# BIH-CEI/napkon-string-matching

Hardware: AMD Instinct MI355X
Metric: pair-comparisons/sec (whole node), N x M all-pairs (higher is better)
Workload: dtype u64; 1 GPU; C3: 200000x200000 strings/GPU (len U[16,64], 37 symbols), fuzzy_match RAW, threshold 0.8; score_func=fuzzy_match, mode=RAW, hits_per_rank=2000, hits_all_ranks=2000, exact_prune=True, hit_ordering=second stream, overlapped with the next step's grid kernel (two hit buffers)

## Files before the change

### napkon-string-matching_amd/csrc/indel_raw_coarse.hpp

```cpp
#pragma once

namespace nsm {

#ifndef NSM_C3C_CAP
#define NSM_C3C_CAP 3
#endif
#ifndef NSM_C3C_FP4
#define NSM_C3C_FP4 1
#endif
#ifndef NSM_C3C_FP4_PERM
#define NSM_C3C_FP4_PERM 1
#endif
#ifndef NSM_C3C_FP4_SPLIT
#define NSM_C3C_FP4_SPLIT 4
#endif
#ifndef NSM_C3C_NT
#define NSM_C3C_NT 4
#endif
#ifndef NSM_C3C_ORFOLD
#define NSM_C3C_ORFOLD (NSM_C3C_FP4 && NSM_C3C_NT % 2 == 0)
#endif
#ifndef NSM_C3C_PIPE
#define NSM_C3C_PIPE (NSM_C3C_NT % (NSM_C3C_ORFOLD ? 4 : 2) == 0)
#endif
#ifndef NSM_C3C_OR_SPLIT
#define NSM_C3C_OR_SPLIT 2
#endif
#ifndef NSM_C3C_LCS_PREFETCH
#define NSM_C3C_LCS_PREFETCH 1
#endif
#ifndef NSM_C3C_EARLY_OUT
#define NSM_C3C_EARLY_OUT 1
#endif
#ifndef NSM_C3C_PERSIST
#define NSM_C3C_PERSIST 0
#endif
#ifndef NSM_C3P_ITEM_ROWS
#define NSM_C3P_ITEM_ROWS 0
#endif
constexpr int kC3cBlock = 32;
constexpr int kC3cRights = NSM_C3C_NT * kC3cBlock;
constexpr int kC3cPipeExtra = NSM_C3C_PIPE ? (NSM_C3C_ORFOLD ? 2 : 1) : 0;
constexpr int kC3cStack = (NSM_C3C_NT + 2 + kC3cPipeExtra) * kWave;
constexpr int kC3cDrainAt = 2 * kWave;
static_assert(NSM_C3C_NT >= 1 && NSM_C3C_NT <= 4, "an entry keeps its tile in 2 bits");
static_assert(NSM_C3C_CAP >= 2 && NSM_C3C_CAP <= 8, "code slots per bucket");

static inline size_t c3c_lds_bytes() {
  return static_cast<size_t>(kWavesPerBlock) * (kC3cStack * 8 + static_cast<size_t>(kC3cRights) * (8 * 4 + 1)) + 136;
}

typedef int c3c_v4i __attribute__((ext_vector_type(4)));
typedef int c3c_v16i __attribute__((ext_vector_type(16)));
typedef int c3c_v8i __attribute__((ext_vector_type(8)));
typedef float c3c_v16f __attribute__((ext_vector_type(16)));

__device__ __forceinline__ uint32_t c3c_ge64(uint32_t w, int k) {
  return (w + static_cast<uint32_t>(0x40 - k) * 0x01010101u) & 0x40404040u;
}


__device__ __forceinline__ int c3c_fp4_scale(const uint4& f0, const uint4& f1) {
  const uint32_t ws[8] = {f0.x, f0.y, f0.z, f0.w, f1.x, f1.y, f1.z, f1.w};
  uint32_t any = 0u;
#pragma unroll
  for (int q = 0; q < 8; ++q) any |= ws[q];
  if ((any & 0xf0f0f0f0u) == 0u) return 0;
  uint32_t top = 0u;
#pragma unroll
  for (int q = 0; q < 8; ++q)
#pragma unroll
    for (int b = 0; b < 4; ++b) top = max(top, (ws[q] >> (8 * b)) & 0xffu);
  return top <= 27u ? 1 : top <= 51u ? 2 : 3;
}
__device__ __forceinline__ void c3c_fp4_right_k0(uint32_t fw, int& m1, int& m2) {
  const uint32_t sel = fw & 0x07070707u;
  const uint32_t big = ((fw >> 3) & 0x01010101u) * 0xffu;
  const uint32_t lo1 = __builtin_amdgcn_perm(0x11111111u, 0x11110100u, sel);
  const uint32_t lo2 = __builtin_amdgcn_perm(0x41312111u, 0x01000000u, sel), hi2 = __builtin_amdgcn_perm(0x71717171u, 0x61615151u, sel);
  m1 = static_cast<int>((big & 0x11111111u) | (~big & lo1));
  m2 = static_cast<int>((big & hi2) | (~big & lo2));
}
__device__ __forceinline__ void c3c_fp4_right_scaled(uint32_t fw, int k, int& m1, int& m2) {
  m1 = static_cast<int>((c3c_ge64(fw, 1) >> 6) | (c3c_ge64(fw, 2) >> 2));
  uint32_t w2 = c3c_ge64(fw, 3) >> 6;
  const uint32_t round_up = (1u << k) - 1u;
#pragma unroll
  for (int b = 0; b < 4; ++b) {
    const uint32_t r = (fw >> (8 * b)) & 0xffu;
    const uint32_t q = (max(r, 3u) - 3u + round_up) >> k;
    w2 |= (static_cast<uint32_t>(0x7777665543210ull >> (4u * q)) & 0xfu) << (8 * b + 4);
  }
  m2 = static_cast<int>(w2);
}
__device__ __forceinline__ void c3c_fp4_left(uint32_t w, int& m1, int& m2) {
#if NSM_C3C_FP4_PERM
  const uint32_t sel = (w + 0x3c3c3c3cu) & 0x43434343u;
  m1 = static_cast<int>(__builtin_amdgcn_perm(0u, 0x44440400u, sel) & 0x44444444u);
  m2 = static_cast<int>(__builtin_amdgcn_perm(0u, 0x04000000u, sel) & 0x44444444u);
#else
  m1 = static_cast<int>(((c3c_ge64(w, 1) >> 4)) | c3c_ge64(w, 2));
  m2 = static_cast<int>(((c3c_ge64(w, 3) >> 4)) | c3c_ge64(w, 4));
#endif
}
__device__ __forceinline__ c3c_v16f c3c_fp4_mfma1(const c3c_v4i& a, const c3c_v4i& b) {
  const c3c_v8i a8 = {a.x, a.y, a.z, a.w, 0, 0, 0, 0}, b8 = {b.x, b.y, b.z, b.w, 0, 0, 0, 0};
  const c3c_v16f zero = {0, 0, 0, 0, 0, 0, 0, 0, 0, 0, 0, 0, 0, 0, 0, 0};
  return __builtin_amdgcn_mfma_scale_f32_32x32x64_f8f6f4(a8, b8, zero, 4, 4, 0, 0, 0, 0);
}
__device__ __forceinline__ c3c_v16f c3c_fp4_mfma2(const c3c_v4i& a, const c3c_v4i& b, const c3c_v16f& acc, int scales, int t) {
  const c3c_v8i a8 = {a.x, a.y, a.z, a.w, 0, 0, 0, 0}, b8 = {b.x, b.y, b.z, b.w, 0, 0, 0, 0};
  switch (t) {
    case 0: return __builtin_amdgcn_mfma_scale_f32_32x32x64_f8f6f4(a8, b8, acc, 4, 4, 0, 0x7f7f7f7f, 0, scales);
    case 1: return __builtin_amdgcn_mfma_scale_f32_32x32x64_f8f6f4(a8, b8, acc, 4, 4, 0, 0x7f7f7f7f, 1, scales);
    case 2: return __builtin_amdgcn_mfma_scale_f32_32x32x64_f8f6f4(a8, b8, acc, 4, 4, 0, 0x7f7f7f7f, 2, scales);
    default: return __builtin_amdgcn_mfma_scale_f32_32x32x64_f8f6f4(a8, b8, acc, 4, 4, 0, 0x7f7f7f7f, 3, scales);
  }
}

constexpr int kC3cPackedRow = 64;
#ifndef NSM_C3C_PACK_MIN_PAIRS
#define NSM_C3C_PACK_MIN_PAIRS 10000000000ll
#endif
static inline bool c3c_pack_pays(long long pairs) { return pairs >= static_cast<long long>(NSM_C3C_PACK_MIN_PAIRS); }
struct c3c_packed_rows {
  c3c_v4i m1, m2;
};
template <bool PACKED>
struct c3c_rows {
  typedef uint4 type;
};
template <>
struct c3c_rows<true> {
  typedef c3c_packed_rows type;
};

__device__ __forceinline__ void c3c_pack_left_unit(const uint32_t* __restrict__ lhist, c3c_v4i* __restrict__ packed, int n_left,
                                                   int u) {
  if (u >= 2 * n_left) return;
  const uint4 w = reinterpret_cast<const uint4*>(lhist)[u];
  const uint32_t ws[4] = {w.x, w.y, w.z, w.w};
  c3c_v4i m1, m2;
#pragma unroll
  for (int q = 0; q < 4; ++q) {
    int a1, a2;
    c3c_fp4_left(ws[q], a1, a2);
    m1[q] = a1;
    m2[q] = a2;
  }
  packed[2 * static_cast<size_t>(u)] = m1;
  packed[2 * static_cast<size_t>(u) + 1] = m2;
}
__global__ __launch_bounds__(kBlock) void c3c_pack_left_kernel(const uint32_t* __restrict__ lhist, c3c_v4i* __restrict__ packed,
                                                               int n_left) {
  c3c_pack_left_unit(lhist, packed, n_left, blockIdx.x * kBlock + threadIdx.x);
}

constexpr int kC3pWindow = 1 << 15;
struct C3pItemParams {
  int n_left, n_right, n_tiles, item_rows, every_row;
  unsigned int cap;
  uint8_t la_lo[65], la_hi[65];
};
__host__ __device__ static inline int c3p_items_of(int rows, int item_rows) {
  const int per_window = (kC3pWindow + item_rows - 1) / item_rows;
  return (rows >> 15) * per_window + ((rows & (kC3pWindow - 1)) + item_rows - 1) / item_rows;
}
constexpr int kC3pQueueBytes = 64;
__host__ __device__ static inline unsigned int* c3p_queue(const char* lpacked) {
  return reinterpret_cast<unsigned int*>(const_cast<char*>(lpacked) - kC3pQueueBytes);
}
__host__ __device__ static inline int4* c3p_item(unsigned int* queue, unsigned int k) {
  return reinterpret_cast<int4*>(queue) - 1 - k;
}
__global__ __launch_bounds__(kBlock) void c3p_prepass_kernel(const uint32_t* __restrict__ lhist, c3c_v4i* __restrict__ packed,
                                                             const int32_t* __restrict__ rlen, const int32_t* __restrict__ lstart,
                                                             unsigned int* __restrict__ queue,
                                                             const C3pItemParams ip, int item_blocks) {
  if (static_cast<int>(blockIdx.x) >= item_blocks) {
    c3c_pack_left_unit(lhist, packed, ip.n_left, (static_cast<int>(blockIdx.x) - item_blocks) * kBlock + static_cast<int>(threadIdx.x));
    return;
  }
  __shared__ unsigned long long s_scan[kBlock];
  const int tid = threadIdx.x;
  auto interval = [&](int t, int& r0) -> int {
    r0 = 0;
    if (ip.every_row) return ip.n_left;
    const int j_a = t * kC3cRights, j_b = min(j_a + kC3cRights, ip.n_right) - 1;
    const int lb_a = min(max(rlen[j_a], 0), 64), lb_b = min(max(rlen[j_b], 0), 64);
    int lo = 65, hi = 0;
    for (int lb = min(lb_a, lb_b); lb <= max(lb_a, lb_b); ++lb) {
      lo = min(lo, static_cast<int>(ip.la_lo[lb]));
      hi = max(hi, static_cast<int>(ip.la_hi[lb]));
    }
    if (hi < lo) return 0;
    r0 = lstart[64 - hi];
    return lstart[64 - lo + 1] - r0;
  };
  unsigned int before = 0u;
  for (int t = tid; t < static_cast<int>(blockIdx.x) * kBlock; t += kBlock) {
    int r0;
    before += static_cast<unsigned int>(c3p_items_of(interval(t, r0), ip.item_rows));
  }
  const int tile = static_cast<int>(blockIdx.x) * kBlock + tid;
  int r0 = 0, rows = 0;
  if (tile < ip.n_tiles) rows = interval(tile, r0);
  const unsigned int own = static_cast<unsigned int>(c3p_items_of(rows, ip.item_rows));
  unsigned long long v = (static_cast<unsigned long long>(before) << 32) | own;
  s_scan[tid] = v;
  __syncthreads();
  for (int d = 1; d < kBlock; d <<= 1) {
    const unsigned long long add = tid >= d ? s_scan[tid - d] : 0ull;
    __syncthreads();
    v += add;
    s_scan[tid] = v;
    __syncthreads();
  }
  const unsigned long long total = s_scan[kBlock - 1];
  const unsigned int carry = static_cast<unsigned int>(total >> 32);
  unsigned int at = carry + static_cast<unsigned int>(v) - own;
  const int per_window = (kC3pWindow + ip.item_rows - 1) / ip.item_rows;
  for (unsigned int k = 0; k < own; ++k, ++at) {
    const int base = r0 + (static_cast<int>(k) / per_window) * kC3pWindow;
    const int first = base + (static_cast<int>(k) % per_window) * ip.item_rows;
    const int end = min(first + ip.item_rows, min(base + kC3pWindow, r0 + rows));
    if (at < ip.cap) *c3p_item(queue, at) = make_int4(tile, first, end, base);
  }
  if (static_cast<int>(blockIdx.x) == item_blocks - 1 && tid == 0) {
    queue[0] = 0u;
    queue[1] = min(carry + static_cast<unsigned int>(total), ip.cap);
  }
}

#ifndef NSM_C3C_OCC
#define NSM_C3C_OCC __attribute__((amdgpu_waves_per_eu((NSM_C3C_ORFOLD && PACKED) ? 4 : 2)))
#endif
template <int NT, int CAP, bool PACKED, bool PERSIST = false>
__global__ __launch_bounds__(kBlock) NSM_C3C_OCC void indel_raw_coarse_kernel(
    const uint8_t* __restrict__ lcodes, const int32_t* __restrict__ llen, const int32_t* __restrict__ lstart,
    const int32_t* __restrict__ lorig, const uint32_t* __restrict__ lhist, const uint8_t* __restrict__ rcodes,
    const int32_t* __restrict__ rlen, const int32_t* __restrict__ rorig, const uint32_t* __restrict__ rhist,
    nsm_hit* __restrict__ hits, unsigned long long* __restrict__ count, const IndelRawParams p,
    const char* __restrict__ lpacked) {
  static_assert(!PACKED || NSM_C3C_FP4, "only the FP4 scan has packed left rows");
  static_assert(!PERSIST || PACKED, "the persistent launch is the packed scan's");
  constexpr int kRights = NT * kC3cBlock;
  static_assert(kC3cDrainAt >= kWave && kC3cDrainAt + (NT + kC3cPipeExtra) * kWave <= kC3cStack,
                "the drain is triggered above kC3cDrainAt entries and runs full passes");
  constexpr bool kOrFold = NSM_C3C_ORFOLD && PACKED;
  constexpr int kFlagHi = 1 << 17, kFlagLo = 1 << 8;
  static_assert(!kOrFold || (NSM_C3C_FP4 && NT % 2 == 0), "the OR fold puts tiles 2 p and 2 p + 1 of the FP4 scan on one accumulator");
  extern __shared__ __attribute__((aligned(16))) unsigned long long s_mem[];
  unsigned long long* s_stack = s_mem;
  uint32_t* s_rh = reinterpret_cast<uint32_t*>(s_stack + kWavesPerBlock * kC3cStack);
  uint8_t* s_rl = reinterpret_cast<uint8_t*>(s_rh + kWavesPerBlock * 8 * kRights);
  uint8_t* s_lcsmin = s_rl + kWavesPerBlock * kRights;
  for (int t = threadIdx.x; t < 132; t += kBlock) s_lcsmin[t] = p.lcsmin[t];
  __syncthreads();

  const int lane = threadIdx.x & (kWave - 1);
  const int wave = threadIdx.x >> 6;
  const int col = lane & (kC3cBlock - 1);
  const int half = lane >> 5;
  int j0 = (blockIdx.x * kWavesPerBlock + wave) * kRights;
  if (!PERSIST && j0 >= p.n_right) return;
  auto lane_again = [&]() -> int {
    int l = lane;
    asm volatile("" : "+v"(l));
    return l;
  };
#if NSM_C3C_EARLY_OUT
  if (!PERSIST && p.zero_need != 0) {
    const int ie = blockIdx.y * p.rows_per_chunk;
    const int la_hi = llen[ie], la_lo = llen[min(p.n_left, ie + p.rows_per_chunk) - 1];
    bool fits = false;
#pragma unroll
    for (int k = 0; k < (kRights + kWave - 1) / kWave; ++k) {
      const int j = j0 + k * kWave + lane;
      if (k * kWave + lane < kRights && j < p.n_right) {
        const int lb = rlen[j];
        const int la = min(max(lb, la_lo), la_hi);
        const int nd = (la == 0 || lb == 0) ? p.zero_need : static_cast<int>(s_lcsmin[la + lb]);
        fits = fits || min(la, lb) >= nd;
      }
    }
    if (!__any(fits)) return;
  }
#endif
  unsigned long long* stack = s_stack + wave * kC3cStack;
  uint32_t* rh_lds = s_rh + wave * 8 * kRights;
  uint8_t* rl_lds = s_rl + wave * kRights;

  bool valid[NT];
  c3c_v4i bfrag[NT][NSM_C3C_FP4 ? 2 : CAP];
  uint32_t bscales = 0u;
  int q_cnt = 0;
  int i0 = 0, ifirst = 0, i1 = 0;
  int it_cur = 0, it_end = 0;
  bool other_tile = true;
  if constexpr (PERSIST) j0 = -1;
  do {
    if constexpr (PERSIST) {
      unsigned int* queue = c3p_queue(lpacked);
      if (it_cur >= it_end) {
        const unsigned int n_items = static_cast<unsigned int>(__builtin_amdgcn_readfirstlane(static_cast<int>(queue[1])));
        unsigned int start = 0u, grain = 0u;
        if (lane == 0) {
          const unsigned int seen = *reinterpret_cast<volatile unsigned int*>(queue);
          const unsigned int left = seen < n_items ? n_items - seen : 0u;
          grain = max(1u, left / (2u * gridDim.x * kWavesPerBlock));
          start = atomicAdd(queue, grain);
        }
        const unsigned int s = static_cast<unsigned int>(__builtin_amdgcn_readfirstlane(static_cast<int>(start)));
        const unsigned int g = static_cast<unsigned int>(__builtin_amdgcn_readfirstlane(static_cast<int>(grain)));
        if (s >= n_items) return;
        it_cur = static_cast<int>(s);
        it_end = static_cast<int>(min(s + g, n_items));
      }
      const int4 it = *c3p_item(queue, static_cast<unsigned int>(it_cur++));
      const int j_it = __builtin_amdgcn_readfirstlane(it.x) * kRights;
      other_tile = j_it != j0;
      j0 = j_it;
      ifirst = __builtin_amdgcn_readfirstlane(it.y);
      i1 = __builtin_amdgcn_readfirstlane(it.z);
      i0 = __builtin_amdgcn_readfirstlane(it.w);
    }
    if (!PERSIST || other_tile) {
      int ln = lane;
      if constexpr (PERSIST) ln = lane_again();
#pragma unroll
      for (int k = 0; k < (kRights + kWave - 1) / kWave; ++k) {
        const int rl = k * kWave + ln;
        if (rl < kRights) {
          const int j = j0 + rl;
          const int jcl = j < p.n_right ? j : p.n_right - 1;
          const uint4* fp = reinterpret_cast<const uint4*>(rhist + static_cast<size_t>(jcl) * 8);
          const uint4 f0 = fp[0], f1 = fp[1];
          uint32_t* dst = rh_lds + rl;
          dst[0 * kRights] = f0.x; dst[1 * kRights] = f0.y; dst[2 * kRights] = f0.z; dst[3 * kRights] = f0.w;
          dst[4 * kRights] = f1.x; dst[5 * kRights] = f1.y; dst[6 * kRights] = f1.z; dst[7 * kRights] = f1.w;
          rl_lds[rl] = static_cast<uint8_t>(j < p.n_right ? rlen[jcl] : 0);
        }
      }
    }
#if NSM_C3C_FP4
    auto scale_base = [](int t) -> uint32_t { return (kOrFold && t % 2 == 0) ? 0x7fu + 9u : 0x7fu; };
    uint32_t bscales1 = 0u;
    if constexpr (kOrFold) {
#pragma unroll
      for (int t = 0; t < NT; ++t) bscales1 |= scale_base(t) << (8 * t);
      asm volatile("" : "+v"(bscales1));
    }
    auto code_tile = [&](int t, const uint4& f, int k) __attribute__((always_inline)) {
      const uint32_t ws[4] = {f.x, f.y, f.z, f.w};
      if (k == 0) {
#pragma unroll
        for (int q = 0; q < 4; ++q) {
          int m1, m2;
          c3c_fp4_right_k0(ws[q], m1, m2);
          bfrag[t][0][q] = m1;
          bfrag[t][1][q] = m2;
        }
      } else {
#pragma unroll
        for (int q = 0; q < 4; ++q) {
          int m1, m2;
          c3c_fp4_right_scaled(ws[q], k, m1, m2);
          bfrag[t][0][q] = m1;
          bfrag[t][1][q] = m2;
        }
      }
    };
    if (!PERSIST || other_tile) {
      bscales = 0u;
      int col_r = col, half_r = half;
      if constexpr (PERSIST) {
        const int l = lane_again();
        col_r = l & (kC3cBlock - 1);
        half_r = l >> 5;
      }
#pragma unroll
      for (int t = 0; t < NT; ++t) {
        const int j = j0 + t * kC3cBlock + col_r;
        valid[t] = j < p.n_right;
        const int jcl = valid[t] ? j : p.n_right - 1;
        const uint4* fp = reinterpret_cast<const uint4*>(rhist + static_cast<size_t>(jcl) * 8);
        const uint4 f0 = fp[0], f1 = fp[1];
        const int k = c3c_fp4_scale(f0, f1);
        bscales |= (scale_base(t) + static_cast<uint32_t>(k)) << (8 * t);
        uint4 f = half_r ? f1 : f0;
        if (!valid[t]) f = make_uint4(0u, 0u, 0u, 0u);
        code_tile(t, f, k);
      }
    }
    auto make_bfrag = [&]() __attribute__((always_inline)) {
      const int l = lane_again();
      const uint32_t* rp0 = rh_lds + (4 * (l >> 5)) * kRights + (l & (kC3cBlock - 1));
#pragma unroll
      for (int t = 0; t < NT; ++t) {
        const uint32_t* rp = rp0 + t * kC3cBlock;
        const int k = static_cast<int>(((bscales >> (8 * t)) & 0xffu) - scale_base(t));
        uint4 f = make_uint4(rp[0], rp[kRights], rp[2 * kRights], rp[3 * kRights]);
        if (!valid[t]) f = make_uint4(0u, 0u, 0u, 0u);
        code_tile(t, f, k);
      }
    };
    __builtin_amdgcn_fence(__ATOMIC_ACQ_REL, "wavefront");
    __builtin_amdgcn_wave_barrier();
#else
    auto code_b = [&](int t, int q, uint32_t fw) {
      const uint32_t full = c3c_ge64(fw, CAP);
#pragma unroll
      for (int s = 0; s < CAP - 1; ++s)
        bfrag[t][s][q] = static_cast<int>((c3c_ge64(fw, s + 1) ^ full) >> 6);
      bfrag[t][CAP - 1][q] = static_cast<int>(full);
    };
#pragma unroll
    for (int t = 0; t < NT; ++t) {
      const int j = j0 + t * kC3cBlock + col;
      valid[t] = j < p.n_right;
      const int jcl = valid[t] ? j : p.n_right - 1;
      uint4 f = reinterpret_cast<const uint4*>(rhist + static_cast<size_t>(jcl) * 8)[half];
      if (!valid[t]) f = make_uint4(0u, 0u, 0u, 0u);
      code_b(t, 0, f.x); code_b(t, 1, f.y); code_b(t, 2, f.z); code_b(t, 3, f.w);
    }
    auto make_bfrag = [&]() {
#pragma unroll
      for (int t = 0; t < NT; ++t) {
        const uint32_t* rp = rh_lds + (4 * half) * kRights + t * kC3cBlock + col;
#pragma unroll
        for (int q = 0; q < 4; ++q) code_b(t, q, valid[t] ? rp[q * kRights] : 0u);
      }
    };
    __builtin_amdgcn_fence(__ATOMIC_ACQ_REL, "wavefront");
    __builtin_amdgcn_wave_barrier();
#endif
    if constexpr (!PERSIST) {
      i0 = ifirst = blockIdx.y * p.rows_per_chunk;
      i1 = min(p.n_left, i0 + p.rows_per_chunk);
    }

    auto need_of = [&](int la, int lb) -> int { return (la == 0 || lb == 0) ? p.zero_need : static_cast<int>(s_lcsmin[la + lb]); };

    const char* chunk = reinterpret_cast<const char*>(lhist + static_cast<size_t>(i0) * 8);
    const char* pchunk = PACKED ? lpacked + static_cast<size_t>(i0) * kC3cPackedRow : nullptr;

    auto drain_pass = [&]() __attribute__((always_inline)) {
      __builtin_amdgcn_fence(__ATOMIC_ACQ_REL, "wavefront");
      __builtin_amdgcn_wave_barrier();
      const int n = min(q_cnt, kWave);
      const int base = q_cnt - n;
      q_cnt = base;
#ifdef NSM_C3C_X_NODRAIN
      return;
#endif
      const int m = lane & 3;
      uint32_t mask = 0;
#pragma nounroll
      for (int s = (n - 1) >> 4; s >= 0; --s) {
        const int e = 16 * s + (lane >> 2);
        const bool active = e < n;
        const unsigned long long ent = stack[base + (active ? e : 0)];
        const int n_rows = active ? static_cast<int>(static_cast<uint32_t>(ent)) : 0;
        const uint32_t ehi = static_cast<uint32_t>(ent >> 32);
        const uint32_t ib_rel = active ? ehi >> 15 : 0u;
        const int r0 = 4 * static_cast<int>((ehi >> 5) & 1u) + m;
        const uint32_t last_r = static_cast<uint32_t>(max(n_rows, 1) - 1);
        uint4 w0[4], w1[4];
#pragma unroll
        for (int g = 0; g < 4; ++g) {
          const uint4* lp = reinterpret_cast<const uint4*>(chunk + (ib_rel + min(static_cast<uint32_t>(r0 + 8 * g), last_r)) * 32u);
          w0[g] = lp[0];
          w1[g] = lp[1];
        }
        const int la = static_cast<int>((ehi >> 8) & 127u);
        const int tl = static_cast<int>((ehi >> 6) & 3u) * kC3cBlock + static_cast<int>(ehi & 31u);
        const int lb = rl_lds[tl];
        uint32_t rq[8];
        {
          const uint32_t* rp = rh_lds + tl;
#pragma unroll
          for (int q = 0; q < 8; ++q) rq[q] = rp[q * kRights];
        }
        const int nd = need_of(la, lb);
        const int budget = (active && min(la, lb) >= nd) ? la + lb - 2 * nd : -1;
        const uint32_t sad0 = ~static_cast<uint32_t>(budget);
#pragma unroll
        for (int g = 3; g >= 0; --g) {
          uint32_t l1 = sad0;
          l1 = __builtin_amdgcn_sad_u8(w0[g].x, rq[0], l1);
          l1 = __builtin_amdgcn_sad_u8(w0[g].y, rq[1], l1);
          l1 = __builtin_amdgcn_sad_u8(w0[g].z, rq[2], l1);
          l1 = __builtin_amdgcn_sad_u8(w0[g].w, rq[3], l1);
          l1 = __builtin_amdgcn_sad_u8(w1[g].x, rq[4], l1);
          l1 = __builtin_amdgcn_sad_u8(w1[g].y, rq[5], l1);
          l1 = __builtin_amdgcn_sad_u8(w1[g].z, rq[6], l1);
          l1 = __builtin_amdgcn_sad_u8(w1[g].w, rq[7], l1);
          if (r0 + 8 * g >= n_rows) l1 = 0u;
          mask = __builtin_amdgcn_alignbit(mask, l1, 31);
        }
      }
#ifdef NSM_C3C_X_NOLCS
      mask = 0u;
#endif
#ifdef NSM_C3C_X_FINEONLY
      mask = p.n_left < 0 ? mask : 0u;
#endif
      unsigned long long todo = __ballot(mask != 0u);
      uint32_t cur = 0u;
      int leader = 0, row_s = 0, j_n = 0, la_n = 0, lb_n = 0;
      auto next_pair = [&]() -> bool {
        if (cur == 0u) {
          if (todo == 0ull) return false;
          leader = __builtin_ctzll(todo);
          todo &= todo - 1ull;
          cur = static_cast<uint32_t>(__builtin_amdgcn_readlane(static_cast<int>(mask), leader));
        }
        const int pos = 31 - __builtin_clz(cur);
        cur &= ~(1u << pos);
        const uint32_t ehi = static_cast<uint32_t>(
            __builtin_amdgcn_readfirstlane(static_cast<int>(stack[base + 16 * (pos >> 2) + (leader >> 2)] >> 32)));
        const int tl = static_cast<int>((ehi >> 6) & 3u) * kC3cBlock + static_cast<int>(ehi & 31u);
        row_s = i0 + static_cast<int>(ehi >> 15) + 8 * (pos & 3) + 4 * static_cast<int>((ehi >> 5) & 1u) + (leader & 3);
        j_n = j0 + tl;
        la_n = static_cast<int>((ehi >> 8) & 127u);
        lb_n = __builtin_amdgcn_readfirstlane(static_cast<int>(rl_lds[tl]));
        return true;
      };
      auto row_units = [&](uint32_t& lc, uint32_t& rc) {
        lc = lcodes[static_cast<size_t>(row_s) * 64 + lane];
        rc = rcodes[static_cast<size_t>(j_n) * 64 + lane];
      };
      uint32_t lc_next = 0, rc_next = 0;
      bool have = next_pair();
      if (NSM_C3C_LCS_PREFETCH && have) row_units(lc_next, rc_next);
      while (have) {
        const int row_c = row_s, j_s = j_n, la_s = la_n, lb_s = lb_n;
        const int need_s = need_of(la_s, lb_s);
        uint32_t lc = lc_next, rc = rc_next;
        if (!NSM_C3C_LCS_PREFETCH) row_units(lc, rc);
        have = next_pair();
        if (NSM_C3C_LCS_PREFETCH && have) row_units(lc_next, rc_next);
        const int lcs = raw_lcs_units(lc, la_s, rc, lb_s, need_s, lane);
#ifdef NSM_C3C_X_COUNTLCS
        if (lane == 0)
#else
        if (lcs >= need_s && lane == 0)
#endif
          emit_hit(hits, p.cap, count, indel_score(la_s, lb_s, lcs), lorig[row_c], rorig[j_s]);
      }
    };
    auto drain_full = [&]() __attribute__((always_inline)) {
      while (q_cnt >= kWave) drain_pass();
      make_bfrag();
    };

    const int c_first = 64 - llen[ifirst];
    const int c_last = 64 - llen[i1 - 1];
    uint32_t lane_off = static_cast<uint32_t>(col * 32 + half * 16);
    if constexpr (PERSIST) {
      const int l = lane_again();
      lane_off = static_cast<uint32_t>((l & (kC3cBlock - 1)) * 32 + (l >> 5) * 16);
    }
    for (int c = c_first; c <= c_last; ++c) {
      const int a = max(ifirst, lstart[c]);
      const int b = min(i1, lstart[c + 1]);
      if (a >= b) continue;
      const int la = 64 - c;
      int need2[2] = {static_cast<int>(kNever), static_cast<int>(kNever)};
      int nm1[NT];
      bool some = false;
      const int l_c = lane_again();
#pragma unroll
      for (int t = 0; t < NT; ++t) {
        const int lb = rl_lds[t * kC3cBlock + (l_c & (kC3cBlock - 1))];
        const int nd = valid[t] ? need_of(la, lb) : static_cast<int>(kNever);
        const bool fits = min(la, lb) >= nd;
        some = some || fits;
#if NSM_C3C_FP4
        if constexpr (kOrFold)
          need2[t & 1] = min(need2[t & 1], fits ? nd : static_cast<int>(kNever));
        else
          nm1[t] = __float_as_int(static_cast<float>(fits ? nd : static_cast<int>(kNever)) - 0.5f);
#else
        nm1[t] = 64 * (fits ? nd : static_cast<int>(kNever)) - 1;
#endif
      }
      if (!__any(some)) continue;
      c3c_v16f bias;
      const float bias1 = __int_as_float(0x4b000000 | ((256 - need2[0]) << 9) | (256 - need2[1]));
      auto make_bias = [&]() {
#pragma unroll
        for (int k = 0; k < 16; ++k) {
          float x;
          asm volatile("v_mov_b32 %0, %1" : "=v"(x) : "v"(bias1));
          bias[k] = x;
        }
      };

      typedef typename c3c_rows<PACKED>::type rows_t;
      const uint32_t last_off = static_cast<uint32_t>(b - 1 - i0) * (PACKED ? 64u : 32u) + static_cast<uint32_t>((l_c >> 5) * (PACKED ? 32 : 16));
      auto load_rows = [&](int i) -> rows_t {
        if constexpr (PACKED) {
          const uint32_t off = min(static_cast<uint32_t>(i - i0) * 64u + 2u * lane_off, last_off);
          const c3c_v4i* pp = reinterpret_cast<const c3c_v4i*>(pchunk + off);
          return c3c_packed_rows{pp[0], pp[1]};
        } else {
          const uint32_t off = min(static_cast<uint32_t>(i - i0) * 32u + lane_off, last_off);
          return *reinterpret_cast<const uint4*>(chunk + off);
        }
      };
#if NSM_C3C_FP4
      typedef c3c_v16f acc_t;
      c3c_v4i afrag[2];
      auto make_afrag = [&](const rows_t& w) {
        if constexpr (!PACKED) {
          const uint32_t ws[4] = {w.x, w.y, w.z, w.w};
#pragma unroll
          for (int q = 0; q < 4; ++q) {
            int m1, m2;
            c3c_fp4_left(ws[q], m1, m2);
            afrag[0][q] = m1;
            afrag[1][q] = m2;
          }
        }
      };
      constexpr int NU = kOrFold ? NT / 2 : NT;
      auto chain = [&](int u, const rows_t& w) -> acc_t {
        if constexpr (kOrFold) {
          acc_t acc = c3c_fp4_mfma2(w.m1, bfrag[2 * u][0], bias, static_cast<int>(bscales1), 2 * u);
          acc = c3c_fp4_mfma2(w.m2, bfrag[2 * u][1], acc, static_cast<int>(bscales), 2 * u);
          acc = c3c_fp4_mfma2(w.m1, bfrag[2 * u + 1][0], acc, static_cast<int>(bscales1), 2 * u + 1);
          return c3c_fp4_mfma2(w.m2, bfrag[2 * u + 1][1], acc, static_cast<int>(bscales), 2 * u + 1);
        } else if constexpr (PACKED) {
          return c3c_fp4_mfma2(w.m2, bfrag[u][1], c3c_fp4_mfma1(w.m1, bfrag[u][0]), static_cast<int>(bscales), u);
        } else {
          return c3c_fp4_mfma2(afrag[1], bfrag[u][1], c3c_fp4_mfma1(afrag[0], bfrag[u][0]), static_cast<int>(bscales), u);
        }
      };
      auto fold = [&](const acc_t& acc) -> int {
        const c3c_v16i bits = __builtin_bit_cast(c3c_v16i, acc);
        if constexpr (kOrFold) {
          int top = bits[0] | bits[1] | bits[2];
#pragma unroll
          for (int k = 3; k < 15; k += 2) top = top | bits[k] | bits[k + 1];
          return (top | bits[15]) & (kFlagHi | kFlagLo);
        } else {
          int top = max(max(bits[0], bits[1]), bits[2]);
#pragma unroll
          for (int k = 3; k < 15; k += 2) top = max(max(top, bits[k]), bits[k + 1]);
          return max(top, bits[15]);
        }
      };
#else
      typedef c3c_v16i acc_t;
      constexpr int NU = NT;
      c3c_v4i afrag[CAP - 1];
      auto make_afrag = [&](const uint4& w) {
#pragma unroll
        for (int s = 0; s < CAP - 1; ++s) {
          afrag[s].x = static_cast<int>(c3c_ge64(w.x, s + 1)); afrag[s].y = static_cast<int>(c3c_ge64(w.y, s + 1));
          afrag[s].z = static_cast<int>(c3c_ge64(w.z, s + 1)); afrag[s].w = static_cast<int>(c3c_ge64(w.w, s + 1));
        }
      };
      auto chain = [&](int t, const uint4& w) -> c3c_v16i {
        c3c_v16i acc = {0, 0, 0, 0, 0, 0, 0, 0, 0, 0, 0, 0, 0, 0, 0, 0};
#pragma unroll
        for (int s = 0; s < CAP - 1; ++s) acc = __builtin_amdgcn_mfma_i32_32x32x32_i8(afrag[s], bfrag[t][s], acc, 0, 0, 0);
        const c3c_v4i last = {static_cast<int>(w.x), static_cast<int>(w.y), static_cast<int>(w.z), static_cast<int>(w.w)};
        return __builtin_amdgcn_mfma_i32_32x32x32_i8(last, bfrag[t][CAP - 1], acc, 0, 0, 0);
      };
      auto fold = [&](const c3c_v16i& acc) -> int {
        int top = max(max(acc[0], acc[1]), acc[2]);
#pragma unroll
        for (int k = 3; k < 15; k += 2) top = max(max(top, acc[k]), acc[k + 1]);
        return max(top, acc[15]);
      };
#endif
      auto push = [&](bool ps, unsigned long long m, int t, int i) {
        if (m == 0ull) return;
#ifdef NSM_C3C_X_COUNTPUSH
        if (lane == 0) atomicAdd(count, static_cast<unsigned long long>(__popcll(m)));
#endif
        if (ps) {
          const int slot = __builtin_amdgcn_mbcnt_hi(static_cast<uint32_t>(m >> 32), __builtin_amdgcn_mbcnt_lo(static_cast<uint32_t>(m), static_cast<uint32_t>(q_cnt)));
          const uint32_t hi = (static_cast<uint32_t>(i - i0) << 15) | (static_cast<uint32_t>(la) << 8) | (static_cast<uint32_t>(t) << 6);
          uint32_t el = static_cast<uint32_t>(lane);
          asm volatile("" : "+v"(el));
          const uint32_t n_rows = static_cast<uint32_t>(min(kC3cBlock, b - i));
          stack[slot] = (static_cast<unsigned long long>(hi | el) << 32) | n_rows;
        }
        q_cnt += __popcll(m);
      };
      auto finish = [&](int top, int u, int i) {
        if constexpr (kOrFold) {
          if (__ballot(top != 0) == 0ull) return;
          const bool hi = (top & kFlagHi) != 0 && valid[2 * u], lo = (top & kFlagLo) != 0 && valid[2 * u + 1];
          push(hi, __ballot(hi), 2 * u, i);
          push(lo, __ballot(lo), 2 * u + 1, i);
        } else {
          const bool ps = top > nm1[u];
          push(ps, __ballot(ps), u, i);
        }
      };
#if NSM_C3C_PIPE
      static_assert(NU % 2 == 0, "unit 0 of the next block takes the accumulator of unit NU: NU must be even (or NSM_C3C_PIPE=0)");
      acc_t acc[2];
      auto block = [&](int i, rows_t& wc, rows_t& wn) __attribute__((always_inline)) -> bool {
        const bool more = i + kC3cBlock < b;
        bool flush = false;
#pragma unroll
        for (int t = 0; t < NU; ++t) {
          if (t + 1 < NU) {
            acc[(t + 1) & 1] = chain(t + 1, wc);
          } else {
            flush = q_cnt > kC3cDrainAt;
            if (kOrFold || (more && !flush)) {
              make_afrag(wn);
              if constexpr (PACKED) asm volatile("" : "+v"(wn.m1), "+v"(wn.m2));
              if (i + 2 * kC3cBlock < b) wc = load_rows(i + 2 * kC3cBlock);
              acc[0] = chain(0, wn);
            }
          }
          const int top = fold(acc[t & 1]);
#if NSM_C3C_FP4
          if constexpr (kOrFold) {
            __builtin_amdgcn_sched_group_barrier(0x008, 1, 0);
            __builtin_amdgcn_sched_group_barrier(0x002, NSM_C3C_OR_SPLIT, 0);
            __builtin_amdgcn_sched_group_barrier(0x008, 1, 0);
            __builtin_amdgcn_sched_group_barrier(0x002, NSM_C3C_OR_SPLIT, 0);
            __builtin_amdgcn_sched_group_barrier(0x008, 1, 0);
            __builtin_amdgcn_sched_group_barrier(0x002, NSM_C3C_OR_SPLIT, 0);
            __builtin_amdgcn_sched_group_barrier(0x008, 1, 0);
            __builtin_amdgcn_sched_group_barrier(0x002, 8 - 3 * NSM_C3C_OR_SPLIT, 0);
          } else {
            __builtin_amdgcn_sched_group_barrier(0x008, 1, 0);
            __builtin_amdgcn_sched_group_barrier(0x002, NSM_C3C_FP4_SPLIT, 0);
            __builtin_amdgcn_sched_group_barrier(0x008, 1, 0);
            __builtin_amdgcn_sched_group_barrier(0x002, 8 - NSM_C3C_FP4_SPLIT, 0);
          }
          if (t + 1 < NU || kOrFold || (more && !flush)) asm volatile("" : "+v"(acc[(t + 1) & 1]));
#else
          __builtin_amdgcn_sched_group_barrier(0x008, 1, 0);
          __builtin_amdgcn_sched_group_barrier(0x002, 4, 0);
          __builtin_amdgcn_sched_group_barrier(0x008, 1, 0);
          __builtin_amdgcn_sched_group_barrier(0x002, 4, 0);
          __builtin_amdgcn_sched_group_barrier(0x008, 1, 0);
#endif
          finish(top, t, i);
        }
        return flush;
      };
      for (int i = a; i < b;) {
        if (q_cnt > kC3cDrainAt)
          drain_full();
        if constexpr (kOrFold) make_bias();
        rows_t w0 = load_rows(i);
        make_afrag(w0);
        rows_t w1;
        if constexpr (PACKED) {
          w1 = load_rows(i + kC3cBlock);
        } else {
          w1 = w0;
          if (i + kC3cBlock < b) w1 = load_rows(i + kC3cBlock);
        }
        acc[0] = chain(0, w0);
        for (;;) {
          const bool f0 = block(i, w0, w1);
          if ((i += kC3cBlock) >= b || f0) break;
          const bool f1 = block(i, w1, w0);
          if ((i += kC3cBlock) >= b || f1) break;
        }
      }
#else
      if constexpr (kOrFold) make_bias();
      rows_t w_next = load_rows(a);
      for (int i = a; i < b; i += kC3cBlock) {
        const rows_t w = w_next;
        if (i + kC3cBlock < b) w_next = load_rows(i + kC3cBlock);
        if (q_cnt > kC3cDrainAt)
          drain_full();
        make_afrag(w);
#pragma unroll
        for (int t = 0; t < NU; ++t) {
          const acc_t acc = chain(t, w);
          finish(fold(acc), t, i);
        }
      }
#endif
    }
    bool keep = false;
    if constexpr (PERSIST) {
      if (it_cur < it_end) {
        const int4 nx = *c3p_item(c3p_queue(lpacked), static_cast<unsigned int>(it_cur));
        keep = __builtin_amdgcn_readfirstlane(nx.x) * kRights == j0 && __builtin_amdgcn_readfirstlane(nx.w) == i0;
      }
    }
    if (!keep) {
      while (q_cnt > 0) drain_pass();
    }
  } while (PERSIST);
}

}
```

Measured before the change: 43480 billion pair-comparisons/s.

## Encode second FP4 histogram plane with finer quarter-step codes in packed scan

Adds a CODES2 encoding, on by default, for the second FP4 operand plane in the packed coarse scan. Left and right histogram counts are mapped through perm-based lookup tables into values with two fractional bits. The OR-fold accumulator fields widen from 9 to 11 bits, and the scale exponents and bias are adjusted to match. The intent is a tighter coarse upper bound on the fuzzy-match score, so fewer candidate pairs reach the expensive exact LCS stage. In exchange, packing and right-fragment construction cost a few more ALU ops, and the wider fields use up headroom in the fp32 accumulator.

Result: faster. 45990 billion pair-comparisons/s, median of 6 (+5.8%).

```diff
diff --git a/napkon-string-matching_amd/csrc/indel_raw_coarse.hpp b/napkon-string-matching_amd/csrc/indel_raw_coarse.hpp
--- a/napkon-string-matching_amd/csrc/indel_raw_coarse.hpp
+++ b/napkon-string-matching_amd/csrc/indel_raw_coarse.hpp
@@ -19,6 +19,9 @@
 #endif
 #ifndef NSM_C3C_ORFOLD
 #define NSM_C3C_ORFOLD (NSM_C3C_FP4 && NSM_C3C_NT % 2 == 0)
+#endif
+#ifndef NSM_C3C_CODES2
+#define NSM_C3C_CODES2 1
 #endif
 #ifndef NSM_C3C_PIPE
 #define NSM_C3C_PIPE (NSM_C3C_NT % (NSM_C3C_ORFOLD ? 4 : 2) == 0)
@@ -102,6 +105,45 @@
   m1 = static_cast<int>(((c3c_ge64(w, 1) >> 4)) | c3c_ge64(w, 2));
   m2 = static_cast<int>(((c3c_ge64(w, 3) >> 4)) | c3c_ge64(w, 4));
 #endif
+}
+constexpr uint32_t kC3cLeft2[4] = {0x04000000u, 0x44342424u, 0x45444444u, 0x47464646u};
+constexpr uint32_t kC3cRight2[4] = {0x01000000u, 0x41414121u, 0x52525151u, 0x53535352u};
+__device__ __forceinline__ uint32_t c3c_codes2_bytes(uint32_t w, const uint32_t (&t)[4]) {
+  const uint32_t sel = w & 0x07070707u;
+  const uint32_t big = ((w >> 3) & 0x01010101u) * 0xffu;
+  return (big & __builtin_amdgcn_perm(t[3], t[2], sel)) | (~big & __builtin_amdgcn_perm(t[1], t[0], sel));
+}
+__device__ __forceinline__ void c3c_fp4_left_packed(uint32_t w, int& m1, int& m2) {
+#if NSM_C3C_CODES2
+  int old2;
+  c3c_fp4_left(w, m1, old2);
+  const uint32_t over = (((w + 0x70707070u) >> 7) & 0x01010101u) * 0xffu;
+  m2 = static_cast<int>(c3c_codes2_bytes((w | over) & 0x0f0f0f0fu, kC3cLeft2));
+#else
+  c3c_fp4_left(w, m1, m2);
+#endif
+}
+__device__ __forceinline__ void c3c_codes2_right_k0(uint32_t fw, int& m1, int& m2) {
+  const uint32_t sel = fw & 0x07070707u;
+  const uint32_t big = ((fw >> 3) & 0x01010101u) * 0xffu;
+  const uint32_t lo1 = __builtin_amdgcn_perm(0x11111111u, 0x11110100u, sel);
+  const uint32_t lo2 = __builtin_amdgcn_perm(kC3cRight2[1], kC3cRight2[0], sel), hi2 = __builtin_amdgcn_perm(kC3cRight2[3], kC3cRight2[2], sel);
+  m1 = static_cast<int>((big & 0x11111111u) | (~big & lo1));
+  m2 = static_cast<int>((big & hi2) | (~big & lo2));
+}
+__device__ __forceinline__ void c3c_codes2_right_scaled(uint32_t fw, int k, int& m1, int& m2) {
+  m1 = static_cast<int>((c3c_ge64(fw, 1) >> 6) | (c3c_ge64(fw, 2) >> 2));
+  const unsigned long long lo = (static_cast<unsigned long long>(kC3cRight2[1]) << 32) | kC3cRight2[0];
+  const unsigned long long hi = (static_cast<unsigned long long>(kC3cRight2[3]) << 32) | kC3cRight2[2];
+  const uint32_t round_up = (1u << k) - 1u;
+  uint32_t w2 = 0u;
+#pragma unroll
+  for (int b = 0; b < 4; ++b) {
+    const uint32_t r = (fw >> (8 * b)) & 0xffu;
+    const uint32_t e = min(2u + ((max(r, 2u) - 2u + round_up) >> k), 15u);
+    w2 |= (static_cast<uint32_t>((e & 8u ? hi : lo) >> (8u * (e & 7u))) & 0xffu) << (8 * b);
+  }
+  m2 = static_cast<int>(w2);
 }
 __device__ __forceinline__ c3c_v16f c3c_fp4_mfma1(const c3c_v4i& a, const c3c_v4i& b) {
   const c3c_v8i a8 = {a.x, a.y, a.z, a.w, 0, 0, 0, 0}, b8 = {b.x, b.y, b.z, b.w, 0, 0, 0, 0};
@@ -144,7 +186,7 @@
 #pragma unroll
   for (int q = 0; q < 4; ++q) {
     int a1, a2;
-    c3c_fp4_left(ws[q], a1, a2);
+    c3c_fp4_left_packed(ws[q], a1, a2);
     m1[q] = a1;
     m2[q] = a2;
   }
@@ -248,7 +290,9 @@
   static_assert(kC3cDrainAt >= kWave && kC3cDrainAt + (NT + kC3cPipeExtra) * kWave <= kC3cStack,
                 "the drain is triggered above kC3cDrainAt entries and runs full passes");
   constexpr bool kOrFold = NSM_C3C_ORFOLD && PACKED;
-  constexpr int kFlagHi = 1 << 17, kFlagLo = 1 << 8;
+  constexpr bool kCodes2 = NSM_C3C_CODES2 && PACKED;
+  constexpr int kFieldBits = kCodes2 ? 11 : 9, kFieldFrac = kCodes2 ? 2 : 0;
+  constexpr int kFlagLo = 1 << (kFieldBits - 1), kFlagHi = kFlagLo << kFieldBits;
   static_assert(!kOrFold || (NSM_C3C_FP4 && NT % 2 == 0), "the OR fold puts tiles 2 p and 2 p + 1 of the FP4 scan on one accumulator");
   extern __shared__ __attribute__((aligned(16))) unsigned long long s_mem[];
   unsigned long long* s_stack = s_mem;
@@ -344,7 +388,9 @@
       }
     }
 #if NSM_C3C_FP4
-    auto scale_base = [](int t) -> uint32_t { return (kOrFold && t % 2 == 0) ? 0x7fu + 9u : 0x7fu; };
+    auto scale_base = [](int t) -> uint32_t {
+      return kOrFold ? 0x7fu + static_cast<uint32_t>(kFieldFrac + (t % 2 == 0 ? kFieldBits : 0)) : 0x7fu;
+    };
     uint32_t bscales1 = 0u;
     if constexpr (kOrFold) {
 #pragma unroll
@@ -357,7 +403,10 @@
 #pragma unroll
         for (int q = 0; q < 4; ++q) {
           int m1, m2;
-          c3c_fp4_right_k0(ws[q], m1, m2);
+          if constexpr (kCodes2)
+            c3c_codes2_right_k0(ws[q], m1, m2);
+          else
+            c3c_fp4_right_k0(ws[q], m1, m2);
           bfrag[t][0][q] = m1;
           bfrag[t][1][q] = m2;
         }
@@ -365,7 +414,10 @@
 #pragma unroll
         for (int q = 0; q < 4; ++q) {
           int m1, m2;
-          c3c_fp4_right_scaled(ws[q], k, m1, m2);
+          if constexpr (kCodes2)
+            c3c_codes2_right_scaled(ws[q], k, m1, m2);
+          else
+            c3c_fp4_right_scaled(ws[q], k, m1, m2);
           bfrag[t][0][q] = m1;
           bfrag[t][1][q] = m2;
         }
@@ -581,14 +633,14 @@
         if constexpr (kOrFold)
           need2[t & 1] = min(need2[t & 1], fits ? nd : static_cast<int>(kNever));
         else
-          nm1[t] = __float_as_int(static_cast<float>(fits ? nd : static_cast<int>(kNever)) - 0.5f);
+          nm1[t] = __float_as_int(static_cast<float>(fits ? nd : static_cast<int>(kNever)) - (kCodes2 ? 0.25f : 0.5f));
 #else
         nm1[t] = 64 * (fits ? nd : static_cast<int>(kNever)) - 1;
 #endif
       }
       if (!__any(some)) continue;
       c3c_v16f bias;
-      const float bias1 = __int_as_float(0x4b000000 | ((256 - need2[0]) << 9) | (256 - need2[1]));
+      const float bias1 = __int_as_float(0x4b000000 | (((256 - need2[0]) << kFieldFrac) << kFieldBits) | ((256 - need2[1]) << kFieldFrac));
       auto make_bias = [&]() {
 #pragma unroll
         for (int k = 0; k < 16; ++k) {
```
